# X-rayLaser/DistributedLLM

Measured on NVIDIA H100. Metric: decode tokens/sec LLaMA-7B Q4_0 seq512 bs1, higher is better.
Workload: dtype q4_0*q8_0->f32

## Files before the change

distributedllm_b200/csrc/common.cuh:

```cuda
#pragma once
#include <cuda_runtime.h>
#include <cuda_fp16.h>
#include <cstdint>
#include <cstdio>
#include <cstdarg>
#include <string>

#include "../../include/b200_slice.h"

namespace b200 {

inline std::string & last_error_ref() { static thread_local std::string e; return e; }
inline int fail(int code, const char * fmt, ...) {
    char buf[1024];
    va_list ap; va_start(ap, fmt); vsnprintf(buf, sizeof buf, fmt, ap); va_end(ap);
    last_error_ref() = buf;
    return code;
}
#define B200_CUDA(expr) do { cudaError_t e_ = (expr); if (e_ != cudaSuccess) \
    return b200::fail(B200_ECUDA, "%s failed: %s (%s:%d)", #expr, cudaGetErrorString(e_), __FILE__, __LINE__); } while (0)

__device__ __forceinline__ float fmul(float a, float b) { return __fmul_rn(a, b); }
__device__ __forceinline__ float fadd(float a, float b) { return __fadd_rn(a, b); }
__device__ __forceinline__ float fsub(float a, float b) { return __fsub_rn(a, b); }
__device__ __forceinline__ float ffma(float a, float b, float c) { return __fmaf_rn(a, b, c); }
__device__ __forceinline__ float h2f(uint16_t h) { return __half2float(__ushort_as_half(h)); }
__device__ __forceinline__ uint16_t f2h(float f) { return __half_as_ushort(__float2half_rn(f)); }

__device__ __forceinline__ uint32_t smem_u32(const void * p) { return (uint32_t) __cvta_generic_to_shared(p); }

__device__ __forceinline__ void mbar_init(uint64_t * bar, uint32_t count) {
    asm volatile("mbarrier.init.shared::cta.b64 [%0], %1;" :: "r"(smem_u32(bar)), "r"(count) : "memory");
}
__device__ __forceinline__ void mbar_fence_init() {
    asm volatile("fence.mbarrier_init.release.cluster;" ::: "memory");
}
__device__ __forceinline__ void mbar_arrive(uint64_t * bar) {
    asm volatile("{ .reg .b64 st; mbarrier.arrive.shared::cta.b64 st, [%0]; }" :: "r"(smem_u32(bar)) : "memory");
}
__device__ __forceinline__ void mbar_arrive_expect_tx(uint64_t * bar, uint32_t bytes) {
    asm volatile("{ .reg .b64 st; mbarrier.arrive.expect_tx.shared::cta.b64 st, [%0], %1; }"
                 :: "r"(smem_u32(bar)), "r"(bytes) : "memory");
}
__device__ __forceinline__ bool mbar_try_wait(uint64_t * bar, uint32_t parity) {
    uint32_t ok;
    asm volatile("{ .reg .pred p; mbarrier.try_wait.parity.shared::cta.b64 p, [%1], %2; selp.u32 %0, 1, 0, p; }"
                 : "=r"(ok) : "r"(smem_u32(bar)), "r"(parity) : "memory");
    return ok != 0;
}
__device__ __forceinline__ void mbar_wait(uint64_t * bar, uint32_t parity) {
    while (!mbar_try_wait(bar, parity)) { }
}
__device__ __forceinline__ void bulk_g2s(void * dst_smem, const void * src_gmem, uint32_t bytes, uint64_t * bar) {
    uint64_t pol;
    asm volatile("createpolicy.fractional.L2::evict_first.b64 %0, 1.0;" : "=l"(pol));
    asm volatile("cp.async.bulk.shared::cluster.global.mbarrier::complete_tx::bytes.L2::cache_hint [%0], [%1], %2, [%3], %4;"
                 :: "r"(smem_u32(dst_smem)), "l"(src_gmem), "r"(bytes), "r"(smem_u32(bar)), "l"(pol) : "memory");
}
__device__ __forceinline__ float4 ldg_keep(const float * p) {
    uint64_t pol; float4 v;
    asm volatile("createpolicy.fractional.L2::evict_last.b64 %0, 1.0;" : "=l"(pol));
    asm volatile("ld.global.L2::cache_hint.v4.f32 {%0, %1, %2, %3}, [%4], %5;"
                 : "=f"(v.x), "=f"(v.y), "=f"(v.z), "=f"(v.w) : "l"(p), "l"(pol));
    return v;
}
__device__ __forceinline__ void grid_dep_wait()   { asm volatile("griddepcontrol.wait;" ::: "memory"); }
__device__ __forceinline__ void grid_dep_launch() { asm volatile("griddepcontrol.launch_dependents;" ::: "memory"); }

__device__ __forceinline__ unsigned long long gtime() { unsigned long long t; asm volatile("mov.u64 %0, %%globaltimer;" : "=l"(t)); return t; }
#define B200_TRACE(ptr, slot) do { if (ptr) (ptr)[((size_t) blockIdx.y * gridDim.x + blockIdx.x) * 8 + (slot)] = b200::gtime(); } while (0)

__device__ __forceinline__ void named_bar_sync(int id, int nthreads) {
    asm volatile("bar.sync %0, %1;" :: "r"(id), "r"(nthreads) : "memory");
}

}
```

distributedllm_b200/csrc/fastgemm2.cuh:

```cuda
#pragma once
#include <cuda.h>

#include "kernels.cuh"

namespace b200 {

struct PrepArgs { const float * x; int ldx; const float * norm_w; uint16_t * xh; int K, N; };

template <bool NORM>
__global__ void __launch_bounds__(256) k_prep_q8_f16(const PrepArgs a) {
    __shared__ double red[8];
    grid_dep_wait();
    const int n = blockIdx.x, tid = threadIdx.x, warp = tid >> 5, lane = tid & 31;
    const float * x = a.x + (size_t) n * a.ldx;
    float scale = 1.f;
    if (NORM) {
        double s = 0.0;
        for (int i = tid; i < a.K; i += 256) s += (double) fmul(x[i], x[i]);
        for (int o = 16; o > 0; o >>= 1) s += __shfl_xor_sync(0xffffffffu, s, o);
        if (lane == 0) red[warp] = s;
        __syncthreads();
        double tot = 0.0;
        for (int i = 0; i < 8; i++) tot += red[i];
        scale = __fdiv_rn(1.0f, __fsqrt_rn(fadd((float)(tot / (double) a.K), 1e-6f)));
    }
    for (int b = warp; b < a.K / 32; b += 8) {
        float v = x[b * 32 + lane];
        if (NORM) v = fmul(fmul(v, scale), a.norm_w[b * 32 + lane]);
        float amax = fabsf(v);
        for (int o = 16; o > 0; o >>= 1) amax = fmaxf(amax, __shfl_xor_sync(0xffffffffu, amax, o));
        const float d = h2f(f2h(__fdiv_rn(amax, 127.f)));
        const float id = amax != 0.f ? __fdiv_rn(127.f, amax) : 0.f;
        const float q = (float) rint_small(fmul(v, id));
        a.xh[(size_t) n * a.K + b * 32 + lane] = f2h(fmul(q, d));
    }
}

__device__ __forceinline__ uint64_t gmma_desc_k_sw128(uint32_t smem_addr) {
    return (uint64_t)((smem_addr & 0x3FFFF) >> 4) | ((uint64_t) 1 << 16) | ((uint64_t) 64 << 32) | ((uint64_t) 1 << 62);
}
__device__ __forceinline__ void fence_proxy_async() { asm volatile("fence.proxy.async.shared::cta;" ::: "memory"); }
__device__ __forceinline__ void wgmma_fence()  { asm volatile("wgmma.fence.sync.aligned;" ::: "memory"); }
__device__ __forceinline__ void wgmma_commit() { asm volatile("wgmma.commit_group.sync.aligned;" ::: "memory"); }
template <int N> __device__ __forceinline__ void wgmma_wait() { asm volatile("wgmma.wait_group.sync.aligned %0;" :: "n"(N) : "memory"); }
__device__ __forceinline__ void acc_fence(float (&d)[64]) {
    #pragma unroll
    for (int i = 0; i < 64; i++) asm volatile("" : "+f"(d[i]) :: "memory");
}
__device__ __forceinline__ void wgmma_m64n128k16(float (&d)[64], uint64_t da, uint64_t db) {
    asm volatile("{ .reg .pred p; setp.ne.b32 p, %66, 0;\n"
                 "wgmma.mma_async.sync.aligned.m64n128k16.f32.f16.f16 {"
                 "%0, %1, %2, %3, %4, %5, %6, %7, %8, %9, %10, %11, %12, %13, %14, %15, "
                 "%16, %17, %18, %19, %20, %21, %22, %23, %24, %25, %26, %27, %28, %29, %30, %31, "
                 "%32, %33, %34, %35, %36, %37, %38, %39, %40, %41, %42, %43, %44, %45, %46, %47, "
                 "%48, %49, %50, %51, %52, %53, %54, %55, %56, %57, %58, %59, %60, %61, %62, %63}, "
                 "%64, %65, p, 1, 1, 0, 0; }"
                 : "+f"(d[0]), "+f"(d[1]), "+f"(d[2]), "+f"(d[3]), "+f"(d[4]), "+f"(d[5]), "+f"(d[6]), "+f"(d[7]),
                   "+f"(d[8]), "+f"(d[9]), "+f"(d[10]), "+f"(d[11]), "+f"(d[12]), "+f"(d[13]), "+f"(d[14]), "+f"(d[15]),
                   "+f"(d[16]), "+f"(d[17]), "+f"(d[18]), "+f"(d[19]), "+f"(d[20]), "+f"(d[21]), "+f"(d[22]), "+f"(d[23]),
                   "+f"(d[24]), "+f"(d[25]), "+f"(d[26]), "+f"(d[27]), "+f"(d[28]), "+f"(d[29]), "+f"(d[30]), "+f"(d[31]),
                   "+f"(d[32]), "+f"(d[33]), "+f"(d[34]), "+f"(d[35]), "+f"(d[36]), "+f"(d[37]), "+f"(d[38]), "+f"(d[39]),
                   "+f"(d[40]), "+f"(d[41]), "+f"(d[42]), "+f"(d[43]), "+f"(d[44]), "+f"(d[45]), "+f"(d[46]), "+f"(d[47]),
                   "+f"(d[48]), "+f"(d[49]), "+f"(d[50]), "+f"(d[51]), "+f"(d[52]), "+f"(d[53]), "+f"(d[54]), "+f"(d[55]),
                   "+f"(d[56]), "+f"(d[57]), "+f"(d[58]), "+f"(d[59]), "+f"(d[60]), "+f"(d[61]), "+f"(d[62]), "+f"(d[63])
                 : "l"(da), "l"(db), "n"(1)
                 : "memory");
}

enum { FG_STORE = 0, FG_RESID = 1, FG_GATE = 2 };

template <int EPI, class Args>
__device__ __forceinline__ void gmma_epilogue(const Args & a, const float (&d)[64], int mt, int m0, int tok0) {
    #pragma unroll
    for (int j = 0; j < 16; j++) {
        #pragma unroll
        for (int c = 0; c < 2; c++) {
            const int tok = tok0 + 8 * j + c;
            if (tok >= a.N) continue;
            if (EPI == FG_GATE) {
                const int row = (mt * 8 + (m0 >> 4)) * 8 + (m0 & 7);
                if (row < a.out_rows) a.y[(size_t) tok * a.ldy + row] = fmul(h2f(a.tsilu[f2h(d[4 * j + c])]), d[4 * j + 2 + c]);
            } else {
                #pragma unroll
                for (int i = 0; i < 2; i++) {
                    const int row = mt * 128 + m0 + 8 * i;
                    float val = d[4 * j + 2 * i + c];
                    if (row < a.out_rows) {
                        if (EPI == FG_RESID) val = fadd(val, a.resid[(size_t) tok * a.ldr + row]);
                        a.y[(size_t) tok * a.ldy + row] = val;
                    }
                }
            }
        }
    }
}

constexpr int kF2M = 128, kF2K = 128;
constexpr int kF2DqWarps = 8;
constexpr int kF2Threads = (kF2DqWarps + 1) * 32;
constexpr int kF2ABytes = kF2M * kF2K * 2;
__host__ __device__ constexpr int f2_raw_bytes(int wt) { return 16 * chunk_bytes(wt); }
__host__ __device__ constexpr int f2_stage_bytes(int wt, int nt) { return ((f2_raw_bytes(wt) + 1023) & ~1023) + kF2ABytes + nt * kF2K * 2; }
__host__ __device__ constexpr int f2_stages(int wt, int nt) { return (nt == 128 && wt == kWT_Q4_0) ? 3 : 2; }
__host__ __device__ constexpr int f2_smem(int wt, int nt) { return f2_stages(wt, nt) * f2_stage_bytes(wt, nt) + 128; }

struct FastGemm2Args {
    PackedW W;
    const float * resid; int ldr;
    float * y; int ldy;
    int N, out_rows;
    const uint16_t * tsilu;
};

__device__ __forceinline__ void tma_load_2d(void * dst, const CUtensorMap * map, int c0, int c1, uint64_t * bar) {
    asm volatile("cp.async.bulk.tensor.2d.shared::cluster.global.mbarrier::complete_tx::bytes [%0], [%1, {%2, %3}], [%4];"
                 :: "r"(smem_u32(dst)), "l"(map), "r"(c0), "r"(c1), "r"(smem_u32(bar)) : "memory");
}

template <int WT, int EPI, int NT>
__global__ void __launch_bounds__(kF2Threads, 1) k_gemm_tc2(const FastGemm2Args a, const __grid_constant__ CUtensorMap xmap) {
    constexpr int CB = (WT == kWT_Q4_0) ? kQ4Chunk : kQ8Chunk;
    constexpr int kF2N = NT, kF2BBytes = NT * kF2K * 2, kF2Stages = f2_stages(WT, NT);
    constexpr int RAW = 16 * CB, RAWP = (RAW + 1023) & ~1023, STAGE = RAWP + kF2ABytes + kF2BBytes;
    extern __shared__ __align__(1024) uint8_t smem[];
    uint64_t * bars = (uint64_t *)(smem + kF2Stages * STAGE);
    uint64_t * tma_full = bars, * stage_free = bars + 3;
    const int tid = threadIdx.x, warp = tid >> 5, lane = tid & 31;
    const int mt = blockIdx.x, nt = blockIdx.y;
    const int nbq = a.W.nbq;
    const int TRp = a.W.TR;
    const int tiles_per_m = 16 / TRp;

    if (tid == 0) {
        for (int s = 0; s < kF2Stages; s++) { mbar_init(&tma_full[s], 1); mbar_init(&stage_free[s], 2); }
        mbar_fence_init();
    }
    __syncthreads();

    if (warp == kF2DqWarps) {
        if (lane == 0) {
            grid_dep_launch();
            grid_dep_wait();
            const uint32_t per_tile = (uint32_t) TRp * CB;
            for (int kb = 0; kb < nbq; kb++) {
                const int s = kb % kF2Stages, use = kb / kF2Stages;
                if (use > 0) mbar_wait(&stage_free[s], (use - 1) & 1);
                uint8_t * stage = smem + (size_t) s * STAGE;
                mbar_arrive_expect_tx(&tma_full[s], (uint32_t)(RAW + kF2BBytes));
                for (int t = 0; t < tiles_per_m; t++) {
                    const uint8_t * src = a.W.data + (long long)(mt * tiles_per_m + t) * a.W.tile_bytes + (size_t) kb * per_tile;
                    bulk_g2s(stage + (size_t) t * per_tile, src, per_tile, &tma_full[s]);
                }
                uint8_t * B = stage + RAWP + kF2ABytes;
                tma_load_2d(B, &xmap, kb * kF2K, nt * kF2N, &tma_full[s]);
                tma_load_2d(B + kF2N * 128, &xmap, kb * kF2K + 64, nt * kF2N, &tma_full[s]);
            }
        }
    } else {
        const int wg = warp >> 2;
        float acc[NT / 128][64];
        #pragma unroll
        for (int n = 0; n < NT / 128; n++)
            #pragma unroll
            for (int i = 0; i < 64; i++) acc[n][i] = 0.f;
        const int r8 = lane >> 2, w = lane & 3;
        for (int kb = 0; kb < nbq; kb++) {
            const int s = kb % kF2Stages, use = kb / kF2Stages;
            uint8_t * stage = smem + (size_t) s * STAGE;
            uint8_t * A = stage + RAWP;
            mbar_wait(&tma_full[s], use & 1);
            #pragma unroll
            for (int gi = 0; gi < 2; gi++) {
                const int g = warp * 2 + gi;
                const uint8_t * ch = stage + (size_t) g * CB;
                const uint4 wv = *(const uint4 *)(ch + lane * 16);
                uint4 wv2 = make_uint4(0, 0, 0, 0); uint2 sc;
                if (WT == kWT_Q8_0) { wv2 = *(const uint4 *)(ch + 512 + lane * 16); sc = *(const uint2 *)(ch + 1024 + r8 * 8); }
                else sc = *(const uint2 *)(ch + 512 + r8 * 8);
                const uint32_t ww[4] = {wv.x, wv.y, wv.z, wv.w};
                const uint32_t ww2[4] = {wv2.x, wv2.y, wv2.z, wv2.w};
                const uint32_t sw[2] = {sc.x, sc.y};
                const int row = g * 8 + r8;
                #pragma unroll
                for (int bq = 0; bq < 4; bq++) {
                    const uint32_t dh = (sw[bq >> 1] >> (16 * (bq & 1))) & 0xFFFFu;
                    const __half2 d2 = __halves2half2(__ushort_as_half((unsigned short) dh), __ushort_as_half((unsigned short) dh));
                    uint32_t lo0, lo1, hi0, hi1;
                    if (WT == kWT_Q4_0) {
                        const uint32_t x = ww[bq] ^ 0x88888888u;
                        const __half2 off = __halves2half2(__ushort_as_half((unsigned short) 0x6408), __ushort_as_half((unsigned short) 0x6408));
                        uint32_t h[4];
                        #pragma unroll
                        for (int i = 0; i < 4; i++) {
                            const uint32_t m = ((x >> (4 * i)) & 0x000F000Fu) | 0x64006400u;
                            const __half2 v = __hmul2(__hsub2(*(const __half2 *) &m, off), d2);
                            h[i] = *(const uint32_t *) &v;
                        }
                        lo0 = __byte_perm(h[0], h[2], 0x5410); lo1 = __byte_perm(h[0], h[2], 0x7632);
                        hi0 = __byte_perm(h[1], h[3], 0x5410); hi1 = __byte_perm(h[1], h[3], 0x7632);
                    } else {
                        const __half2 off = __halves2half2(__ushort_as_half((unsigned short) 0x6480), __ushort_as_half((unsigned short) 0x6480));
                        const uint32_t ul = ww[bq] ^ 0x80808080u, uh = ww2[bq] ^ 0x80808080u;
                        const uint32_t m0 = __byte_perm(ul, 0x64646464u, 0x4140), m1 = __byte_perm(ul, 0x64646464u, 0x4342);
                        const uint32_t m2 = __byte_perm(uh, 0x64646464u, 0x4140), m3 = __byte_perm(uh, 0x64646464u, 0x4342);
                        const __half2 v0 = __hmul2(__hsub2(*(const __half2 *) &m0, off), d2), v1 = __hmul2(__hsub2(*(const __half2 *) &m1, off), d2);
                        const __half2 v2 = __hmul2(__hsub2(*(const __half2 *) &m2, off), d2), v3 = __hmul2(__hsub2(*(const __half2 *) &m3, off), d2);
                        lo0 = *(const uint32_t *) &v0; lo1 = *(const uint32_t *) &v1; hi0 = *(const uint32_t *) &v2; hi1 = *(const uint32_t *) &v3;
                    }
                    const int klo = bq * 32 + 4 * w, khi = klo + 16;
                    {
                        const int sub = klo >> 6, kk = klo & 63, c8 = kk >> 3, within = (kk & 7) * 2;
                        *(uint2 *)(A + sub * (kF2M * 128) + row * 128 + ((c8 ^ (row & 7)) << 4) + within) = make_uint2(lo0, lo1);
                    }
                    {
                        const int sub = khi >> 6, kk = khi & 63, c8 = kk >> 3, within = (kk & 7) * 2;
                        *(uint2 *)(A + sub * (kF2M * 128) + row * 128 + ((c8 ^ (row & 7)) << 4) + within) = make_uint2(hi0, hi1);
                    }
                }
            }
            fence_proxy_async();
            named_bar_sync(1 + wg, 128);
            const uint32_t a_addr = smem_u32(A) + wg * (64 * 128), b_addr = smem_u32(stage + RAWP + kF2ABytes);
            wgmma_fence();
            #pragma unroll
            for (int n = 0; n < NT / 128; n++) acc_fence(acc[n]);
            #pragma unroll
            for (int k16 = 0; k16 < 8; k16++) {
                const uint32_t off = (k16 & 3) * 32;
                #pragma unroll
                for (int n = 0; n < NT / 128; n++)
                    wgmma_m64n128k16(acc[n], gmma_desc_k_sw128(a_addr + (k16 >> 2) * (kF2M * 128) + off),
                                     gmma_desc_k_sw128(b_addr + (k16 >> 2) * (kF2N * 128) + n * (128 * 128) + off));
            }
            wgmma_commit();
            wgmma_wait<1>();
            #pragma unroll
            for (int n = 0; n < NT / 128; n++) acc_fence(acc[n]);
            if (kb > 0 && (tid & 127) == 0) mbar_arrive(&stage_free[(kb - 1) % kF2Stages]);
        }
        wgmma_wait<0>();
        #pragma unroll
        for (int n = 0; n < NT / 128; n++) acc_fence(acc[n]);
        #pragma unroll
        for (int n = 0; n < NT / 128; n++)
            gmma_epilogue<EPI>(a, acc[n], mt, wg * 64 + (warp & 3) * 16 + r8, nt * kF2N + n * 128 + 2 * w);
    }
}

}
```

distributedllm_b200/csrc/kernels.cuh:

```cuda
#pragma once
#include "common.cuh"

namespace b200 {

constexpr int kWT_F16 = 1, kWT_Q4_0 = 2, kWT_Q4_1 = 3, kWT_Q5_0 = 6, kWT_Q5_1 = 7, kWT_Q8_0 = 8;
constexpr int kQ4Chunk = 576, kQ41Chunk = 640, kQ50Chunk = 704, kQ51Chunk = 768, kQ8Chunk = 1088;
constexpr int kWPC = 4;
constexpr int kConsumers = kWPC * 32;
constexpr int kQS = 4;
constexpr float kMagic = 12582912.0f;
constexpr int kMagicI = 0x4B400000;

struct WtTraits {
    int block_bytes;
    int chunk_bytes;
    bool is_signed;
    bool min_plane;
    bool high_plane;
    bool q8_1;
    float act_scale;
};
__host__ __device__ constexpr WtTraits wt_traits(int wt) {
    return wt == kWT_Q4_0 ? WtTraits{18, kQ4Chunk, true, false, false, false, 0.0625f}
         : wt == kWT_Q4_1 ? WtTraits{20, kQ41Chunk, false, true, false, true, 0.0625f}
// ... 153 lines not shown
}

enum { PRO_PLAIN = 0, PRO_NORM = 1, PRO_PREQ = 2 };
enum { EPI_STORE = 0, EPI_RESID = 1, EPI_GATE = 2, EPI_GATEQ = 3, EPI_RESID_NQ = 4, EPI_RESID_SEND = 5 };

struct GemvArgs {
    PackedW W;
    const float * x;      int ldx;
    const float * norm_w;
    const int * aq_in; const float * da_in;
    int in_soff, out_soff;
    const float * resid;  int ldr;
    float * y;            int ldy;
    int * aq_out; float * da_out; int out_nbq; float out_dscale;
    const float * nq_norm_w; int * nq_counter; double * nq_partial;
    int N;
    int out_rows;
    const uint16_t * tsilu;
    int NS;
    unsigned long long * trace;
    int pre_stages;
    int dbg_nomath;
    MailboxHdr * mb_mine;
    uint2 * mb_peer_inbox; size_t mb_slot_elems;
};

__host__ __device__ inline size_t act_bytes_per_col(int nbq, int wt) { return (size_t) nbq * (128 + 16 + (wt_q8_1(wt) ? 16 : 0)); }


__device__ __forceinline__ double widen_nonneg(float f) {
    const uint32_t u = __float_as_uint(f);
    if (u - 0x00800000u < 0x7F000000u) return __hiloint2double((int)((u >> 3) + 0x38000000u), (int)(u << 29));
    return (double) f;
}
__device__ __forceinline__ int rint_small(float x) { return __float_as_int(fadd(x, kMagic)) - kMagicI; }

__device__ __forceinline__ int dp4a_us(uint32_t a, int b, int c) {
    int d; asm("dp4a.u32.s32 %0, %1, %2, %3;" : "=r"(d) : "r"(a), "r"(b), "r"(c)); return d;
}

__device__ __forceinline__ void warp_quant_block(float v, int lane, int * aq_col, float * da_col, int b, float dscale, int soff = 0) {
    float amax = fabsf(v);
    #pragma unroll
    for (int o = 16; o > 0; o >>= 1) amax = fmaxf(amax, __shfl_xor_sync(0xffffffffu, amax, o));
    const float dq = __fdiv_rn(amax, 127.f);
    const float d = soff ? dq : h2f(f2h(dq));
    const float id = amax != 0.f ? __fdiv_rn(127.f, amax) : 0.f;
    const int qv = rint_small(fmul(v, id));
    uint32_t pk = ((uint32_t)(qv & 0xFF)) << (8 * (lane & 3));
    pk |= __shfl_xor_sync(0xffffffffu, pk, 1);
    pk |= __shfl_xor_sync(0xffffffffu, pk, 2);
    if ((lane & 3) == 0) {
        const int w = lane >> 2;
        aq_col[(b >> 2) * 32 + (w & 3) * 8 + (b & 3) * 2 + (w >> 2)] = (int) pk;
    }
    if (lane == 0) da_col[b] = fmul(d, dscale);
    if (soff) {
        int qs = qv;
        #pragma unroll
        for (int o = 16; o > 0; o >>= 1) qs += __shfl_xor_sync(0xffffffffu, qs, o);
        if (lane == 0) da_col[soff + b] = fmul(d, (float) qs);
    }
}

template <int WT>
__device__ __forceinline__ void thread_quant_block(const float (&v)[32], int * an, float * dn, int b, int rot = 0, float * sn = nullptr) {
    constexpr bool Q81 = wt_q8_1(WT);
    float m[8];
    #pragma unroll
    for (int j = 0; j < 8; j++) m[j] = fmaxf(fmaxf(fabsf(v[j]), fabsf(v[j + 8])), fmaxf(fabsf(v[j + 16]), fabsf(v[j + 24])));
    const float amax = fmaxf(fmaxf(fmaxf(m[0], m[1]), fmaxf(m[2], m[3])), fmaxf(fmaxf(m[4], m[5]), fmaxf(m[6], m[7])));
    const float dq = __fdiv_rn(amax, 127.f);
    const float d = Q81 ? dq : h2f(f2h(dq));
    const float id = amax != 0.f ? __fdiv_rn(127.f, amax) : 0.f;
    dn[b] = wt_nibbles(WT) ? fmul(d, wt_act_scale(WT)) : d;
    int * dst = an + (b >> 2) * 32 + (b & 3) * 2;
    int qsum = 0;
    #pragma unroll
    for (int w = 0; w < 8; w++) {
        uint32_t pk = 0;
        #pragma unroll
        for (int j = 0; j < 4; j++) {
            const int qv = rint_small(fmul(v[w*4 + j], id));
            if (Q81) qsum += qv;
            pk |= ((uint32_t)(qv & 0xFF)) << (8 * j);
        }
        const int ww = (w + rot) & 7;
        dst[(ww & 3) * 8 + (ww >> 2)] = (int) pk;
    }
    if (Q81) sn[b] = fmul(d, (float) qsum);
}

template <int WT, int G, int NC, int PRO, int EPI, bool RING>
__global__ void __launch_bounds__(kConsumers + 32) k_gemv(const GemvArgs a) {
    constexpr int CB = chunk_bytes(WT);
    constexpr bool Q41 = wt_q8_1(WT);
    constexpr bool Q5 = wt_traits(WT).high_plane;
    constexpr int SOFF = wt_scale_off(WT), MOFF = wt_min_off(WT);
    constexpr int TR = kWPC * G;
    extern __shared__ __align__(128) uint8_t smem[];
    const int nbq = a.W.nbq, K = a.W.K, nb = a.W.nb;
    const int NS = a.NS;
    constexpr int stage_bytes = kQS * TR * CB;
    uint8_t * ring = smem;
    int * a_s = (int *)(smem + (RING ? (size_t) NS * stage_bytes : 0));
    float * da_s = (float *)((uint8_t *) a_s + (size_t) NC * nbq * 128);
    float * sa_s = da_s + (size_t) NC * nbq * 4;
    uint64_t * full = (uint64_t *)((uint8_t *) da_s + (size_t) NC * nbq * (Q41 ? 32 : 16));
    uint64_t * empty = full + 16;
    uint64_t * actbar = empty + 16;
    double * red = (double *)(actbar + 2);
    float * gq = (float *)(red + kWPC);
    float * xs = gq + NC * 32;

    const int tid = threadIdx.x, warp = tid >> 5, lane = tid & 31;
    const int col0 = blockIdx.y * NC;
    const int n_stage = nbq / kQS;

    if (tid == 0) {
        B200_TRACE(a.trace, 0);
        if (RING) for (int s = 0; s < NS; s++) { mbar_init(&full[s], 1); mbar_init(&empty[s], kWPC); }
        mbar_init(actbar, 1);
        mbar_init(actbar + 1, kWPC);
        mbar_fence_init();
    }
    __syncthreads();

    if (RING && warp == kWPC) {
        if (lane == 0) {
            int slot = 0, use = 0, issued = 0;
            for (int tile = blockIdx.x; tile < a.W.n_tiles; tile += gridDim.x) {
                const uint8_t * src = a.W.data + (long long) tile * a.W.tile_bytes;
                for (int s = 0; s < n_stage; s++) {
                    if (issued == a.pre_stages) mbar_wait(actbar + 1, 0);
                    issued++;
                    if (use > 0) mbar_wait(&empty[slot], (use - 1) & 1);
                    mbar_arrive_expect_tx(&full[slot], (uint32_t) stage_bytes);
                    bulk_g2s(ring + (size_t) slot * stage_bytes, src + (size_t) s * stage_bytes, (uint32_t) stage_bytes, &full[slot]);
                    if (++slot == NS) { slot = 0; use++; }
                }
            }
            if (issued <= a.pre_stages) mbar_wait(actbar + 1, 0);
            grid_dep_launch();
            B200_TRACE(a.trace, 4);
        }
        return;
    }

    float wn[32];
    if (PRO == PRO_NORM && nb <= kConsumers) {
        #pragma unroll
        for (int j = 0; j < 8; j++) {
            const float4 u = tid < nb ? ldg_keep(a.norm_w + tid * 32 + (((NC == 1 ? tid : 0) + j) & 7) * 4) : make_float4(0.f, 0.f, 0.f, 0.f);
            wn[j*4] = u.x; wn[j*4+1] = u.y; wn[j*4+2] = u.z; wn[j*4+3] = u.w;
        }
    }
    grid_dep_wait();
    if (!RING && tid == 0) grid_dep_launch();
    if (tid == 0) B200_TRACE(a.trace, 1);

    const int ncols = min(NC, a.N - col0);
    bool gate_done = false;
    if (PRO == PRO_PREQ) {
        gate_done = true;
        if (tid == 0) {
            const uint32_t b1 = (uint32_t) ncols * nbq * 128, b2 = (uint32_t) ncols * nbq * 16;
            mbar_arrive_expect_tx(actbar, b1 + b2 + (Q41 ? b2 : 0u));
            bulk_g2s(a_s, a.aq_in + (size_t) col0 * nbq * 32, b1, actbar);
            bulk_g2s(da_s, a.da_in + (size_t) col0 * nbq * 4, b2, actbar);
            if (Q41) bulk_g2s(sa_s, a.da_in + a.in_soff + (size_t) col0 * nbq * 4, b2, actbar);
        }
        if (RING && lane == 0) mbar_arrive(actbar + 1);
        for (int n = ncols; n < NC; n++) {
            for (int i = tid; i < nbq * 32; i += kConsumers) a_s[(size_t) n * nbq * 32 + i] = 0;
            for (int i = tid; i < nbq * 4; i += kConsumers) { da_s[(size_t) n * nbq * 4 + i] = 0.f; if (Q41) sa_s[(size_t) n * nbq * 4 + i] = 0.f; }
        }
        mbar_wait(actbar, 0);
    } else {
        for (int n = 0; n < NC; n++) {
            int * an = a_s + (size_t) n * nbq * 32;
            float * dn = da_s + (size_t) n * nbq * 4;
            float * sn = sa_s + (size_t) n * nbq * 4;
            if (n >= ncols) {
                for (int i = tid; i < nbq * 32; i += kConsumers) an[i] = 0;
                for (int i = tid; i < nbq * 4; i += kConsumers) { dn[i] = 0.f; if (Q41) sn[i] = 0.f; }
                continue;
            }
            const float * x = a.x + (size_t)(col0 + n) * a.ldx;
            for (int b = nb + tid; b < nbq * 4; b += kConsumers) {
                int * dst = an + (b >> 2) * 32 + (b & 3) * 2;
                for (int w = 0; w < 4; w++) { dst[w * 8] = 0; dst[w * 8 + 1] = 0; }
                dn[b] = 0.f;
                if (Q41) sn[b] = 0.f;
            }
            if (PRO == PRO_NORM && nb <= kConsumers) {
                float v[32];
                const bool own = tid < nb;
                const int rot = NC == 1 ? (tid & 7) : 0;
                if (NC == 1) {
                    if (tid == 0) { mbar_arrive_expect_tx(actbar, (uint32_t) K * 4); bulk_g2s(xs, x, (uint32_t) K * 4, actbar); }
                    if (RING && lane == 0) { gate_done = true; mbar_arrive(actbar + 1); }
                    mbar_wait(actbar, 0);
                    #pragma unroll
                    for (int j = 0; j < 8; j++) {
                        const float4 t = own ? *(const float4 *)(xs + tid * 32 + ((j + rot) & 7) * 4) : make_float4(0.f, 0.f, 0.f, 0.f);
                        v[j*4] = t.x; v[j*4+1] = t.y; v[j*4+2] = t.z; v[j*4+3] = t.w;
                    }
                } else {
                    #pragma unroll
                    for (int j = 0; j < 8; j++) {
                        const float4 t = own ? *(const float4 *)(x + tid * 32 + j * 4) : make_float4(0.f, 0.f, 0.f, 0.f);
                        v[j*4] = t.x; v[j*4+1] = t.y; v[j*4+2] = t.z; v[j*4+3] = t.w;
                    }
                    if (RING && n == ncols - 1 && lane == 0) { gate_done = true; mbar_arrive(actbar + 1); }
                }
                double s4[4] = {0.0, 0.0, 0.0, 0.0};
                #pragma unroll
                for (int j = 0; j < 32; j++) s4[j & 3] += widen_nonneg(fmul(v[j], v[j]));
                double s = (s4[0] + s4[1]) + (s4[2] + s4[3]);
                if (tid == 0) B200_TRACE(a.trace, 5);
                for (int o = 16; o > 0; o >>= 1) s += __shfl_xor_sync(0xffffffffu, s, o);
                if (lane == 0) red[warp] = s;
                named_bar_sync(1, kConsumers);
                const double tot = (red[0] + red[1]) + (red[2] + red[3]);
                named_bar_sync(1, kConsumers);
                const float scale = __fdiv_rn(1.0f, __fsqrt_rn(fadd((float)(tot / (double) K), 1e-6f)));
                if (tid == 0) B200_TRACE(a.trace, 6);
                if (own) {
                    #pragma unroll
                    for (int j = 0; j < 32; j++) v[j] = fmul(fmul(v[j], scale), wn[j]);
                    thread_quant_block<WT>(v, an, dn, tid, rot, sn);
                }
            } else {
                float scale = 1.0f;
                if (PRO == PRO_NORM) {
                    double s = 0.0;
                    for (int i = tid * 4; i < K; i += kConsumers * 4) {
                        const float4 v = *(const float4 *)(x + i);
                        s += (double) fmul(v.x, v.x); s += (double) fmul(v.y, v.y);
                        s += (double) fmul(v.z, v.z); s += (double) fmul(v.w, v.w);
                    }
                    for (int o = 16; o > 0; o >>= 1) s += __shfl_xor_sync(0xffffffffu, s, o);
                    if (lane == 0) red[warp] = s;
                    named_bar_sync(1, kConsumers);
                    const double tot = (red[0] + red[1]) + (red[2] + red[3]);
                    named_bar_sync(1, kConsumers);
                    scale = __fdiv_rn(1.0f, __fsqrt_rn(fadd((float)(tot / (double) K), 1e-6f)));
                }
                for (int b = tid; b < nb; b += kConsumers) {
                    float v[32];
                    #pragma unroll
                    for (int j = 0; j < 8; j++) {
                        float4 t = *(const float4 *)(x + b * 32 + j * 4);
                        if (PRO == PRO_NORM) {
                            const float4 wv = *(const float4 *)(a.norm_w + b * 32 + j * 4);
                            t.x = fmul(fmul(t.x, scale), wv.x); t.y = fmul(fmul(t.y, scale), wv.y);
                            t.z = fmul(fmul(t.z, scale), wv.z); t.w = fmul(fmul(t.w, scale), wv.w);
                        }
                        v[j*4] = t.x; v[j*4+1] = t.y; v[j*4+2] = t.z; v[j*4+3] = t.w;
                    }
                    thread_quant_block<WT>(v, an, dn, b, 0, sn);
                }
            }
        }
    }
    if (RING && lane == 0 && !gate_done) mbar_arrive(actbar + 1);
    named_bar_sync(1, kConsumers);
    if (tid == 0) B200_TRACE(a.trace, 2);

    const int r = lane >> 2, w = lane & 3;
    int slot = 0, phase = 0;
#ifdef B200_TRACE_WAITS
    long long dbg_wait = 0, dbg_t0 = a.trace ? clock64() : 0;
#endif
    uint2 * send_slot = nullptr; int send_seq = 0;
    if (EPI == EPI_RESID_SEND) {
        send_seq = a.mb_mine->seq_out + 1;
        if (lane == 0) mb_wait_slot_free(a.mb_mine, send_seq);
        __syncwarp();
        send_slot = a.mb_peer_inbox + (size_t)(send_seq & (kMbSlots - 1)) * a.mb_slot_elems;
    }
    for (int tile = blockIdx.x; tile < a.W.n_tiles; tile += gridDim.x) {
        float acc[G][NC][2];
        float summ[G][NC];
        #pragma unroll
        for (int g = 0; g < G; g++)
            #pragma unroll
            for (int n = 0; n < NC; n++) { acc[g][n][0] = 0.f; acc[g][n][1] = 0.f; summ[g][n] = 0.f; }
        const uint8_t * gsrc = a.W.data + (long long) tile * a.W.tile_bytes;

        for (int s = 0; s < n_stage; s++) {
            const uint8_t * base;
            if (RING) {
#ifdef B200_TRACE_WAITS
                if (a.trace) { const long long c0 = clock64(); mbar_wait(&full[slot], phase); dbg_wait += clock64() - c0; }
                else
#endif
                mbar_wait(&full[slot], phase);
                base = ring + (size_t) slot * stage_bytes;
            } else {
                base = gsrc + (size_t) s * stage_bytes;
            }
            base += (size_t)(warp * G) * CB;
            if (!a.dbg_nomath)
            #pragma unroll
            for (int qi = 0; qi < kQS; qi++) {
                const int Q = s * kQS + qi;
                uint4 wv[G], wv2[G]; uint2 sc[G], mc[G]; uint32_t hw[G];
                #pragma unroll
                for (int g = 0; g < G; g++) {
                    const uint8_t * ch = base + (size_t)(qi * TR + g) * CB;
                    wv[g] = *(const uint4 *)(ch + lane * 16);
                    if (WT == kWT_Q8_0) wv2[g] = *(const uint4 *)(ch + 512 + lane * 16);
                    sc[g] = *(const uint2 *)(ch + SOFF + r * 8);
                    mc[g] = Q41 ? *(const uint2 *)(ch + MOFF + r * 8) : make_uint2(0u, 0u);
                    hw[g] = Q5 ? *(const uint32_t *)(ch + 512 + lane * 4) : 0u;
                }
                #pragma unroll
                for (int n = 0; n < NC; n++) {
                    const int4 * ap = (const int4 *)(a_s + (size_t) n * nbq * 32 + Q * 32 + w * 8);
                    const int4 a01 = ap[0], a23 = ap[1];
                    const float4 dav = *(const float4 *)(da_s + (size_t) n * nbq * 4 + Q * 4);
                    const int alo[4] = {a01.x, a01.z, a23.x, a23.z};
                    const int ahi[4] = {a01.y, a01.w, a23.y, a23.w};
                    const float da[4] = {dav.x, dav.y, dav.z, dav.w};
                    float sa[4] = {0.f, 0.f, 0.f, 0.f};
                    if (Q41) { const float4 sav = *(const float4 *)(sa_s + (size_t) n * nbq * 4 + Q * 4); sa[0] = sav.x; sa[1] = sav.y; sa[2] = sav.z; sa[3] = sav.w; }
                    #pragma unroll
                    for (int g = 0; g < G; g++) {
                        const uint32_t ww[4] = {wv[g].x, wv[g].y, wv[g].z, wv[g].w};
                        const uint32_t ww2[4] = {wv2[g].x, wv2[g].y, wv2[g].z, wv2[g].w};
                        const uint32_t sw[2] = {sc[g].x, sc[g].y};
                        const uint32_t mw[2] = {mc[g].x, mc[g].y};
                        #pragma unroll
                        for (int bq = 0; bq < 4; bq++) {
                            const uint16_t dh = (uint16_t)(sw[bq >> 1] >> (16 * (bq & 1)));
                            const float D = fmul(h2f(dh), da[bq]);
                            float f0, f1;
                            if (Q41) {
                                const uint16_t mh = (uint16_t)(mw[bq >> 1] >> (16 * (bq & 1)));
                                summ[g][n] = fadd(summ[g][n], fmul(h2f(mh), sa[bq]));
                                uint32_t lo, hi;
                                if (Q5) {
                                    lo = ((ww[bq] << 3) & 0x78787878u) | spread4_hi((hw[g] >> (8 * bq)) & 15u);
                                    hi = ((ww[bq] >> 1) & 0x78787878u) | spread4_hi((hw[g] >> (8 * bq + 4)) & 15u);
                                } else { lo = (ww[bq] << 4) & 0xF0F0F0F0u; hi = ww[bq] & 0xF0F0F0F0u; }
                                f0 = fadd(__int_as_float(dp4a_us(lo, alo[bq], kMagicI)), -kMagic);
                                f1 = fadd(__int_as_float(dp4a_us(hi, ahi[bq], kMagicI)), -kMagic);
                            } else {
                                int lo, hi;
                                if (WT == kWT_Q4_0) { lo = (int)((ww[bq] << 4) & 0xF0F0F0F0u); hi = (int)(ww[bq] & 0xF0F0F0F0u); }
                                else if (Q5) {
                                    lo = (int)(((ww[bq] << 3) & 0x78787878u) | (spread4_hi((hw[g] >> (8 * bq)) & 15u) ^ 0x80808080u));
                                    hi = (int)(((ww[bq] >> 1) & 0x78787878u) | (spread4_hi((hw[g] >> (8 * bq + 4)) & 15u) ^ 0x80808080u));
                                }
                                else                { lo = (int) ww[bq]; hi = (int) ww2[bq]; }
                                f0 = fadd(__int_as_float(__dp4a(lo, alo[bq], kMagicI)), -kMagic);
                                f1 = fadd(__int_as_float(__dp4a(hi, ahi[bq], kMagicI)), -kMagic);
                            }
                            acc[g][n][0] = ffma(D, f0, acc[g][n][0]);
                            acc[g][n][1] = ffma(D, f1, acc[g][n][1]);
                        }
                    }
                }
            }
            if (RING) {
                __syncwarp();
                if (lane == 0) mbar_arrive(&empty[slot]);
                if (++slot == NS) { slot = 0; phase ^= 1; }
            }
        }

        float res[G][NC];
        #pragma unroll
        for (int g = 0; g < G; g++)
            #pragma unroll
            for (int n = 0; n < NC; n++) {
                float t = fadd(acc[g][n][0], acc[g][n][1]);
                t = fadd(t, __shfl_xor_sync(0xffffffffu, t, 2));
                t = fadd(t, __shfl_xor_sync(0xffffffffu, t, 1));
                res[g][n] = Q41 ? fadd(t, summ[g][n]) : t;
            }
        if (EPI == EPI_GATE || EPI == EPI_GATEQ) {
            const int row = (tile * kWPC + warp) * 8 + r;
            if (w == 0) {
                #pragma unroll
                for (int n = 0; n < NC; n++) {
                    const float gv = fmul(h2f(a.tsilu[f2h(res[0][n])]), res[G - 1][n]);
                    if (EPI == EPI_GATEQ) gq[n * 32 + warp * 8 + r] = row < a.out_rows ? gv : 0.f;
                    else if (row < a.out_rows && n < ncols) a.y[(size_t)(col0 + n) * a.ldy + row] = gv;
                }
            }
            if (EPI == EPI_GATEQ) {
                named_bar_sync(1, kConsumers);
                for (int n = warp; n < ncols; n += kWPC)
                    warp_quant_block(gq[n * 32 + lane], lane, a.aq_out + (size_t)(col0 + n) * a.out_nbq * 32,
                                     a.da_out + (size_t)(col0 + n) * a.out_nbq * 4, tile, a.out_dscale, a.out_soff);
                named_bar_sync(1, kConsumers);
            }
        } else if (w == 0) {
            #pragma unroll
            for (int g = 0; g < G; g++) {
                const int row = ((tile * kWPC + warp) * G + g) * 8 + r;
                if (row < a.out_rows) {
                    #pragma unroll
                    for (int n = 0; n < NC; n++) {
                        if (n < ncols) {
                            float v = res[g][n];
                            if (EPI == EPI_RESID || EPI == EPI_RESID_NQ || EPI == EPI_RESID_SEND) v = fadd(v, a.resid[(size_t)(col0 + n) * a.ldr + row]);
                            a.y[(size_t)(col0 + n) * a.ldy + row] = v;
                            if (EPI == EPI_RESID_SEND) st_ll(send_slot + row, v, send_seq);
                            if (EPI == EPI_RESID_NQ) gq[n * 32 + warp * 8 + r] = v;
                        }
                    }
                }
            }
        }
    }
    if (EPI == EPI_RESID_NQ) {
        named_bar_sync(1, kConsumers);
        if (warp == 0) {
            const int tile = blockIdx.x, nt = (int) gridDim.x;
            for (int n = 0; n < ncols; n++) {
                const float val = gq[n * 32 + lane];
                double s = widen_nonneg(fmul(val, val));
                for (int o = 16; o > 0; o >>= 1) s += __shfl_xor_sync(0xffffffffu, s, o);
                double * part = a.nq_partial + ((size_t) blockIdx.y * NC + n) * nt;
                if (lane == 0) part[tile] = s;
            }
            int * cnt = a.nq_counter + 2 * blockIdx.y;
            if (lane == 0) {
                __threadfence();
                atomicAdd(cnt, 1);
                while (*(volatile int *) cnt < nt) { }
                __threadfence();
            }
            __syncwarp();
            const int row = tile * 32 + lane;
            for (int n = 0; n < ncols; n++) {
                const double * part = a.nq_partial + ((size_t) blockIdx.y * NC + n) * nt;
                double s = 0.0;
                for (int i = lane; i < nt; i += 32) s += __ldcg(part + i);
                for (int o = 16; o > 0; o >>= 1) s += __shfl_xor_sync(0xffffffffu, s, o);
                const float scale = __fdiv_rn(1.0f, __fsqrt_rn(fadd((float)(s / (double) a.out_rows), 1e-6f)));
                const float val = gq[n * 32 + lane];
                const float wv = row < a.out_rows ? a.nq_norm_w[row] : 0.f;
                warp_quant_block(fmul(fmul(val, scale), wv), lane, a.aq_out + (size_t)(col0 + n) * a.out_nbq * 32,
                                 a.da_out + (size_t)(col0 + n) * a.out_nbq * 4, tile, a.out_dscale, a.out_soff);
            }
            if (lane == 0) {
                if (atomicAdd(cnt + 1, 1) == nt - 1) { cnt[0] = 0; cnt[1] = 0; }
            }
        }
    }
    if (tid == 0) B200_TRACE(a.trace, 3);
#ifdef B200_TRACE_WAITS
    if (tid == 0 && a.trace)
        a.trace[((size_t) blockIdx.y * gridDim.x + blockIdx.x) * 8 + 7] = ((unsigned long long) dbg_wait << 32) | (unsigned long long)((clock64() - dbg_t0) & 0xFFFFFFFFll);
#endif
}

struct NormQuantArgs {
    const float * x; int ldx; const float * norm_w; int K;
    int * aq; float * da; int nbq;
    int soff;
};

template <int WT>
__global__ void __launch_bounds__(256) k_norm_quant(const NormQuantArgs a) {
    __shared__ double red[8];
    const int n = blockIdx.x, tid = threadIdx.x, warp = tid >> 5, lane = tid & 31, nb = a.K / 32;
    if (tid == 0) grid_dep_launch();
    grid_dep_wait();
    const float * x = a.x + (size_t) n * a.ldx;
    double s = 0.0;
    for (int b = tid; b < nb; b += 256) {
        #pragma unroll
        for (int j = 0; j < 8; j++) {
            const float4 t = *(const float4 *)(x + b * 32 + j * 4);
            s += widen_nonneg(fmul(t.x, t.x)); s += widen_nonneg(fmul(t.y, t.y));
            s += widen_nonneg(fmul(t.z, t.z)); s += widen_nonneg(fmul(t.w, t.w));
        }
    }
    for (int o = 16; o > 0; o >>= 1) s += __shfl_xor_sync(0xffffffffu, s, o);
    if (lane == 0) red[warp] = s;
    __syncthreads();
    double tot = 0.0;
    #pragma unroll
    for (int i = 0; i < 8; i++) tot += red[i];
    const float scale = __fdiv_rn(1.0f, __fsqrt_rn(fadd((float)(tot / (double) a.K), 1e-6f)));
    int * an = a.aq + (size_t) n * a.nbq * 32;
    float * dn = a.da + (size_t) n * a.nbq * 4;
    for (int b = tid; b < nb; b += 256) {
        float v[32];
        #pragma unroll
        for (int j = 0; j < 8; j++) {
            const float4 t = *(const float4 *)(x + b * 32 + j * 4);
            const float4 wv = *(const float4 *)(a.norm_w + b * 32 + j * 4);
            v[j*4]   = fmul(fmul(t.x, scale), wv.x); v[j*4+1] = fmul(fmul(t.y, scale), wv.y);
            v[j*4+2] = fmul(fmul(t.z, scale), wv.z); v[j*4+3] = fmul(fmul(t.w, scale), wv.w);
        }
        thread_quant_block<WT>(v, an, dn, b, 0, dn + a.soff);
    }
}

struct GemvF16Args {
    const uint16_t * W;
    const uint16_t * tail;
    int rows, K;
    const float * x; int ldx; const float * norm_w;
    const float * resid; int ldr;
    float * y; int ldy; int N;
    const uint16_t * tsilu;
    const uint16_t * W2; const uint16_t * tail2;
};

template <int PRO, int EPI>
__global__ void __launch_bounds__(256) k_gemv_f16(const GemvF16Args a) {
    extern __shared__ __align__(16) uint8_t smem[];
    uint16_t * xh = (uint16_t *) smem;
    __shared__ double red[8];
    const int tid = threadIdx.x, warp = tid >> 5, lane = tid & 31, K = a.K;
    const int col = blockIdx.y;
    grid_dep_wait();
    const float * x = a.x + (size_t) col * a.ldx;
    float scale = 1.0f;
    if (PRO == PRO_NORM) {
        double s = 0.0;
        for (int i = tid; i < K; i += 256) s += (double) fmul(x[i], x[i]);
        for (int o = 16; o > 0; o >>= 1) s += __shfl_xor_sync(0xffffffffu, s, o);
        if (lane == 0) red[warp] = s;
        __syncthreads();
        double tot = 0.0;
        for (int i = 0; i < 8; i++) tot += red[i];
        scale = __fdiv_rn(1.0f, __fsqrt_rn(fadd((float)(tot / (double) K), 1e-6f)));
    }
    for (int i = tid; i < K; i += 256) {
        float v = x[i];
        if (PRO == PRO_NORM) v = fmul(fmul(v, scale), a.norm_w[i]);
        xh[i] = f2h(v);
    }
    __syncthreads();
    const int nchunk = K / 32, nc8 = (nchunk + 7) / 8, ntail = K & 31;
    for (int row = blockIdx.x * 8 + warp; row < a.rows; row += gridDim.x * 8) {
        float res[2] = {0.f, 0.f};
        #pragma unroll
        for (int m = 0; m < (EPI == EPI_GATE ? 2 : 1); m++) {
            const uint16_t * Wm = m ? a.W2 : a.W;
            const uint16_t * tl = m ? a.tail2 : a.tail;
            float acc = 0.f;
            const uint4 * wp = (const uint4 *)(Wm + ((size_t) row * nc8 * 32 + lane) * 8);
            constexpr int U = 4;
            for (int c8 = 0; c8 < nc8; c8 += U) {
                uint4 v[U];
                #pragma unroll
                for (int q = 0; q < U; q++) v[q] = c8 + q < nc8 ? __ldcs(wp + (size_t)(c8 + q) * 32) : make_uint4(0, 0, 0, 0);
                #pragma unroll
                for (int q = 0; q < U; q++) {
                    const uint32_t u[4] = {v[q].x, v[q].y, v[q].z, v[q].w};
                    #pragma unroll
                    for (int j = 0; j < 8; j++) {
                        const int c = (c8 + q) * 8 + j;
                        if (c < nchunk) {
                            const uint16_t wh = (uint16_t)(u[j >> 1] >> (16 * (j & 1)));
                            acc = ffma(h2f(wh), h2f(xh[c * 32 + lane]), acc);
                        }
                    }
                }
            }
            acc = fadd(acc, __shfl_xor_sync(0xffffffffu, acc, 16));
            acc = fadd(acc, __shfl_xor_sync(0xffffffffu, acc, 8));
            acc = fadd(acc, __shfl_xor_sync(0xffffffffu, acc, 4));
            acc = fadd(acc, __shfl_xor_sync(0xffffffffu, acc, 1));
            acc = fadd(acc, __shfl_xor_sync(0xffffffffu, acc, 2));
            double sumf = (double) acc;
            for (int i = 0; i < ntail; i++)
                sumf += (double) fmul(h2f(tl[(size_t) row * ntail + i]), h2f(xh[nchunk * 32 + i]));
            res[m] = (float) sumf;
        }
        if (lane == 0) {
            float v = res[0];
            if (EPI == EPI_RESID) v = fadd(v, a.resid[(size_t) col * a.ldr + row]);
            if (EPI == EPI_GATE)  v = fmul(h2f(a.tsilu[f2h(res[0])]), res[1]);
            a.y[(size_t) col * a.ldy + row] = v;
        }
    }
}

template <int PRO, int EPI, int NC>
__global__ void __launch_bounds__(256) k_gemv_f16_mc(const GemvF16Args a) {
    static_assert(NC == 4 || NC == 8, "columns per CTA");
    extern __shared__ __align__(16) uint8_t smem[];
    float * xf = (float *) smem;
    __shared__ double red[8];
    const int tid = threadIdx.x, warp = tid >> 5, lane = tid & 31, K = a.K;
    const int col0 = blockIdx.y * NC, ncols = min(NC, a.N - col0);
    grid_dep_wait();
    for (int n = 0; n < NC; n++) {
        if (n >= ncols) { for (int i = tid; i < K; i += 256) xf[(size_t) i * NC + n] = 0.f; continue; }
        const float * x = a.x + (size_t)(col0 + n) * a.ldx;
        float scale = 1.0f;
        if (PRO == PRO_NORM) {
            double s = 0.0;
            for (int i = tid; i < K; i += 256) s += (double) fmul(x[i], x[i]);
            for (int o = 16; o > 0; o >>= 1) s += __shfl_xor_sync(0xffffffffu, s, o);
            __syncthreads();
            if (lane == 0) red[warp] = s;
            __syncthreads();
            double tot = 0.0;
            for (int i = 0; i < 8; i++) tot += red[i];
            scale = __fdiv_rn(1.0f, __fsqrt_rn(fadd((float)(tot / (double) K), 1e-6f)));
        }
        for (int i = tid; i < K; i += 256) {
            float v = x[i];
            if (PRO == PRO_NORM) v = fmul(fmul(v, scale), a.norm_w[i]);
            xf[(size_t) i * NC + n] = h2f(f2h(v));
        }
    }
    __syncthreads();
    const int nchunk = K / 32, nc8 = (nchunk + 7) / 8, ntail = K & 31;
    for (int row0 = (blockIdx.x * 8 + warp) * 2; row0 < a.rows; row0 += gridDim.x * 16) {
        const bool two = row0 + 1 < a.rows;
        float res[2][2][NC];
        #pragma unroll
        for (int m = 0; m < (EPI == EPI_GATE ? 2 : 1); m++) {
            const uint16_t * Wm = m ? a.W2 : a.W;
            const uint16_t * tl = m ? a.tail2 : a.tail;
            float acc[2][NC];
            #pragma unroll
            for (int n = 0; n < NC; n++) { acc[0][n] = 0.f; acc[1][n] = 0.f; }
            const uint4 * wp0 = (const uint4 *)(Wm + ((size_t) row0 * nc8 * 32 + lane) * 8);
            const uint4 * wp1 = (const uint4 *)(Wm + ((size_t)(two ? row0 + 1 : row0) * nc8 * 32 + lane) * 8);
            constexpr int U = 2;
            uint4 v0[U], v1[U];
            #pragma unroll
            for (int q = 0; q < U; q++) {
                v0[q] = q < nc8 ? __ldg(wp0 + (size_t) q * 32) : make_uint4(0, 0, 0, 0);
                v1[q] = q < nc8 ? __ldg(wp1 + (size_t) q * 32) : make_uint4(0, 0, 0, 0);
            }
            for (int c8 = 0; c8 < nc8; c8 += U) {
                uint4 n0[U], n1[U];
                #pragma unroll
                for (int q = 0; q < U; q++) {
                    n0[q] = c8 + U + q < nc8 ? __ldg(wp0 + (size_t)(c8 + U + q) * 32) : make_uint4(0, 0, 0, 0);
                    n1[q] = c8 + U + q < nc8 ? __ldg(wp1 + (size_t)(c8 + U + q) * 32) : make_uint4(0, 0, 0, 0);
                }
                #pragma unroll
                for (int q = 0; q < U; q++) {
                    const uint32_t u0[4] = {v0[q].x, v0[q].y, v0[q].z, v0[q].w};
                    const uint32_t u1[4] = {v1[q].x, v1[q].y, v1[q].z, v1[q].w};
                    #pragma unroll
                    for (int j = 0; j < 8; j++) {
                        const int c = (c8 + q) * 8 + j;
                        if (c < nchunk) {
                            const float w0 = h2f((uint16_t)(u0[j >> 1] >> (16 * (j & 1))));
                            const float w1 = h2f((uint16_t)(u1[j >> 1] >> (16 * (j & 1))));
                            const float4 * xp = (const float4 *)(xf + (size_t)(c * 32 + lane) * NC);
                            #pragma unroll
                            for (int n4 = 0; n4 < NC / 4; n4++) {
                                const float4 xv = xp[n4];
                                acc[0][n4*4]   = ffma(w0, xv.x, acc[0][n4*4]);   acc[0][n4*4+1] = ffma(w0, xv.y, acc[0][n4*4+1]);
                                acc[0][n4*4+2] = ffma(w0, xv.z, acc[0][n4*4+2]); acc[0][n4*4+3] = ffma(w0, xv.w, acc[0][n4*4+3]);
                                acc[1][n4*4]   = ffma(w1, xv.x, acc[1][n4*4]);   acc[1][n4*4+1] = ffma(w1, xv.y, acc[1][n4*4+1]);
                                acc[1][n4*4+2] = ffma(w1, xv.z, acc[1][n4*4+2]); acc[1][n4*4+3] = ffma(w1, xv.w, acc[1][n4*4+3]);
                            }
                        }
                    }
                }
                #pragma unroll
                for (int q = 0; q < U; q++) { v0[q] = n0[q]; v1[q] = n1[q]; }
            }
            #pragma unroll
            for (int rr = 0; rr < 2; rr++)
// ... 808 lines not shown
```

Measured before the change: 554.3.

## Release ring slot early after batching shared-memory weight loads in GEMV

For the single-column (decode) ring-buffered path, each warp now loads several quant groups of weights from the shared-memory stage into registers at once. It then releases the stage's empty barrier, with a proxy fence, before doing the math on the last group. This lets the producer's bulk copy into that slot start sooner and overlap with the remaining compute. The cost is higher register pressure from holding LQ groups of weights live, which could lower occupancy.

```diff
diff --git a/distributedllm_b200/csrc/common.cuh b/distributedllm_b200/csrc/common.cuh
--- a/distributedllm_b200/csrc/common.cuh
+++ b/distributedllm_b200/csrc/common.cuh
@@ -42,6 +42,7 @@
     asm volatile("{ .reg .b64 st; mbarrier.arrive.expect_tx.shared::cta.b64 st, [%0], %1; }"
                  :: "r"(smem_u32(bar)), "r"(bytes) : "memory");
 }
+__device__ __forceinline__ void fence_proxy_async() { asm volatile("fence.proxy.async.shared::cta;" ::: "memory"); }
 __device__ __forceinline__ bool mbar_try_wait(uint64_t * bar, uint32_t parity) {
     uint32_t ok;
     asm volatile("{ .reg .pred p; mbarrier.try_wait.parity.shared::cta.b64 p, [%1], %2; selp.u32 %0, 1, 0, p; }"
diff --git a/distributedllm_b200/csrc/fastgemm2.cuh b/distributedllm_b200/csrc/fastgemm2.cuh
--- a/distributedllm_b200/csrc/fastgemm2.cuh
+++ b/distributedllm_b200/csrc/fastgemm2.cuh
@@ -39,7 +39,6 @@
 __device__ __forceinline__ uint64_t gmma_desc_k_sw128(uint32_t smem_addr) {
     return (uint64_t)((smem_addr & 0x3FFFF) >> 4) | ((uint64_t) 1 << 16) | ((uint64_t) 64 << 32) | ((uint64_t) 1 << 62);
 }
-__device__ __forceinline__ void fence_proxy_async() { asm volatile("fence.proxy.async.shared::cta;" ::: "memory"); }
 __device__ __forceinline__ void wgmma_fence()  { asm volatile("wgmma.fence.sync.aligned;" ::: "memory"); }
 __device__ __forceinline__ void wgmma_commit() { asm volatile("wgmma.commit_group.sync.aligned;" ::: "memory"); }
 template <int N> __device__ __forceinline__ void wgmma_wait() { asm volatile("wgmma.wait_group.sync.aligned %0;" :: "n"(N) : "memory"); }
diff --git a/distributedllm_b200/csrc/kernels.cuh b/distributedllm_b200/csrc/kernels.cuh
--- a/distributedllm_b200/csrc/kernels.cuh
+++ b/distributedllm_b200/csrc/kernels.cuh
@@ -479,73 +479,83 @@
                 base = gsrc + (size_t) s * stage_bytes;
             }
             base += (size_t)(warp * G) * CB;
-            if (!a.dbg_nomath)
-            #pragma unroll
-            for (int qi = 0; qi < kQS; qi++) {
-                const int Q = s * kQS + qi;
-                uint4 wv[G], wv2[G]; uint2 sc[G], mc[G]; uint32_t hw[G];
-                #pragma unroll
-                for (int g = 0; g < G; g++) {
-                    const uint8_t * ch = base + (size_t)(qi * TR + g) * CB;
-                    wv[g] = *(const uint4 *)(ch + lane * 16);
-                    if (WT == kWT_Q8_0) wv2[g] = *(const uint4 *)(ch + 512 + lane * 16);
-                    sc[g] = *(const uint2 *)(ch + SOFF + r * 8);
-                    mc[g] = Q41 ? *(const uint2 *)(ch + MOFF + r * 8) : make_uint2(0u, 0u);
-                    hw[g] = Q5 ? *(const uint32_t *)(ch + 512 + lane * 4) : 0u;
-                }
-                #pragma unroll
-                for (int n = 0; n < NC; n++) {
-                    const int4 * ap = (const int4 *)(a_s + (size_t) n * nbq * 32 + Q * 32 + w * 8);
-                    const int4 a01 = ap[0], a23 = ap[1];
-                    const float4 dav = *(const float4 *)(da_s + (size_t) n * nbq * 4 + Q * 4);
-                    const int alo[4] = {a01.x, a01.z, a23.x, a23.z};
-                    const int ahi[4] = {a01.y, a01.w, a23.y, a23.w};
-                    const float da[4] = {dav.x, dav.y, dav.z, dav.w};
-                    float sa[4] = {0.f, 0.f, 0.f, 0.f};
-                    if (Q41) { const float4 sav = *(const float4 *)(sa_s + (size_t) n * nbq * 4 + Q * 4); sa[0] = sav.x; sa[1] = sav.y; sa[2] = sav.z; sa[3] = sav.w; }
-                    #pragma unroll
-                    for (int g = 0; g < G; g++) {
-                        const uint32_t ww[4] = {wv[g].x, wv[g].y, wv[g].z, wv[g].w};
-                        const uint32_t ww2[4] = {wv2[g].x, wv2[g].y, wv2[g].z, wv2[g].w};
-                        const uint32_t sw[2] = {sc[g].x, sc[g].y};
-                        const uint32_t mw[2] = {mc[g].x, mc[g].y};
-                        #pragma unroll
-                        for (int bq = 0; bq < 4; bq++) {
-                            const uint16_t dh = (uint16_t)(sw[bq >> 1] >> (16 * (bq & 1)));
-                            const float D = fmul(h2f(dh), da[bq]);
-                            float f0, f1;
-                            if (Q41) {
-                                const uint16_t mh = (uint16_t)(mw[bq >> 1] >> (16 * (bq & 1)));
-                                summ[g][n] = fadd(summ[g][n], fmul(h2f(mh), sa[bq]));
-                                uint32_t lo, hi;
-                                if (Q5) {
-                                    lo = ((ww[bq] << 3) & 0x78787878u) | spread4_hi((hw[g] >> (8 * bq)) & 15u);
-                                    hi = ((ww[bq] >> 1) & 0x78787878u) | spread4_hi((hw[g] >> (8 * bq + 4)) & 15u);
-                                } else { lo = (ww[bq] << 4) & 0xF0F0F0F0u; hi = ww[bq] & 0xF0F0F0F0u; }
-                                f0 = fadd(__int_as_float(dp4a_us(lo, alo[bq], kMagicI)), -kMagic);
-                                f1 = fadd(__int_as_float(dp4a_us(hi, ahi[bq], kMagicI)), -kMagic);
-                            } else {
-                                int lo, hi;
-                                if (WT == kWT_Q4_0) { lo = (int)((ww[bq] << 4) & 0xF0F0F0F0u); hi = (int)(ww[bq] & 0xF0F0F0F0u); }
-                                else if (Q5) {
-                                    lo = (int)(((ww[bq] << 3) & 0x78787878u) | (spread4_hi((hw[g] >> (8 * bq)) & 15u) ^ 0x80808080u));
-                                    hi = (int)(((ww[bq] >> 1) & 0x78787878u) | (spread4_hi((hw[g] >> (8 * bq + 4)) & 15u) ^ 0x80808080u));
-                                }
-                                else                { lo = (int) ww[bq]; hi = (int) ww2[bq]; }
-                                f0 = fadd(__int_as_float(__dp4a(lo, alo[bq], kMagicI)), -kMagic);
-                                f1 = fadd(__int_as_float(__dp4a(hi, ahi[bq], kMagicI)), -kMagic);
-                            }
-                            acc[g][n][0] = ffma(D, f0, acc[g][n][0]);
-                            acc[g][n][1] = ffma(D, f1, acc[g][n][1]);
-                        }
-                    }
-                }
-            }
-            if (RING) {
+            constexpr bool early = RING && NC == 1;
+            constexpr int LQ = early ? kQS / G : 1;
+            auto release = [&] {
+                if (early) fence_proxy_async();
                 __syncwarp();
                 if (lane == 0) mbar_arrive(&empty[slot]);
                 if (++slot == NS) { slot = 0; phase ^= 1; }
-            }
+            };
+            if (!a.dbg_nomath)
+            #pragma unroll
+            for (int q0 = 0; q0 < kQS; q0 += LQ) {
+                uint4 wv[LQ][G], wv2[LQ][G]; uint2 sc[LQ][G], mc[LQ][G]; uint32_t hw[LQ][G];
+                #pragma unroll
+                for (int l = 0; l < LQ; l++)
+                    #pragma unroll
+                    for (int g = 0; g < G; g++) {
+                        const uint8_t * ch = base + (size_t)((q0 + l) * TR + g) * CB;
+                        wv[l][g] = *(const uint4 *)(ch + lane * 16);
+                        if (WT == kWT_Q8_0) wv2[l][g] = *(const uint4 *)(ch + 512 + lane * 16);
+                        sc[l][g] = *(const uint2 *)(ch + SOFF + r * 8);
+                        mc[l][g] = Q41 ? *(const uint2 *)(ch + MOFF + r * 8) : make_uint2(0u, 0u);
+                        hw[l][g] = Q5 ? *(const uint32_t *)(ch + 512 + lane * 4) : 0u;
+                    }
+                #pragma unroll
+                for (int l = 0; l < LQ; l++) {
+                    const int Q = s * kQS + q0 + l;
+                    if (early && q0 + LQ == kQS && l == LQ - 1) release();
+                    #pragma unroll
+                    for (int n = 0; n < NC; n++) {
+                        const int4 * ap = (const int4 *)(a_s + (size_t) n * nbq * 32 + Q * 32 + w * 8);
+                        const int4 a01 = ap[0], a23 = ap[1];
+                        const float4 dav = *(const float4 *)(da_s + (size_t) n * nbq * 4 + Q * 4);
+                        const int alo[4] = {a01.x, a01.z, a23.x, a23.z};
+                        const int ahi[4] = {a01.y, a01.w, a23.y, a23.w};
+                        const float da[4] = {dav.x, dav.y, dav.z, dav.w};
+                        float sa[4] = {0.f, 0.f, 0.f, 0.f};
+                        if (Q41) { const float4 sav = *(const float4 *)(sa_s + (size_t) n * nbq * 4 + Q * 4); sa[0] = sav.x; sa[1] = sav.y; sa[2] = sav.z; sa[3] = sav.w; }
+                        #pragma unroll
+                        for (int g = 0; g < G; g++) {
+                            const uint32_t ww[4] = {wv[l][g].x, wv[l][g].y, wv[l][g].z, wv[l][g].w};
+                            const uint32_t ww2[4] = {wv2[l][g].x, wv2[l][g].y, wv2[l][g].z, wv2[l][g].w};
+                            const uint32_t sw[2] = {sc[l][g].x, sc[l][g].y};
+                            const uint32_t mw[2] = {mc[l][g].x, mc[l][g].y};
+                            #pragma unroll
+                            for (int bq = 0; bq < 4; bq++) {
+                                const uint16_t dh = (uint16_t)(sw[bq >> 1] >> (16 * (bq & 1)));
+                                const float D = fmul(h2f(dh), da[bq]);
+                                float f0, f1;
+                                if (Q41) {
+                                    const uint16_t mh = (uint16_t)(mw[bq >> 1] >> (16 * (bq & 1)));
+                                    summ[g][n] = fadd(summ[g][n], fmul(h2f(mh), sa[bq]));
+                                    uint32_t lo, hi;
+                                    if (Q5) {
+                                        lo = ((ww[bq] << 3) & 0x78787878u) | spread4_hi((hw[l][g] >> (8 * bq)) & 15u);
+                                        hi = ((ww[bq] >> 1) & 0x78787878u) | spread4_hi((hw[l][g] >> (8 * bq + 4)) & 15u);
+                                    } else { lo = (ww[bq] << 4) & 0xF0F0F0F0u; hi = ww[bq] & 0xF0F0F0F0u; }
+                                    f0 = fadd(__int_as_float(dp4a_us(lo, alo[bq], kMagicI)), -kMagic);
+                                    f1 = fadd(__int_as_float(dp4a_us(hi, ahi[bq], kMagicI)), -kMagic);
+                                } else {
+                                    int lo, hi;
+                                    if (WT == kWT_Q4_0) { lo = (int)((ww[bq] << 4) & 0xF0F0F0F0u); hi = (int)(ww[bq] & 0xF0F0F0F0u); }
+                                    else if (Q5) {
+                                        lo = (int)(((ww[bq] << 3) & 0x78787878u) | (spread4_hi((hw[l][g] >> (8 * bq)) & 15u) ^ 0x80808080u));
+                                        hi = (int)(((ww[bq] >> 1) & 0x78787878u) | (spread4_hi((hw[l][g] >> (8 * bq + 4)) & 15u) ^ 0x80808080u));
+                                    }
+                                    else                { lo = (int) ww[bq]; hi = (int) ww2[bq]; }
+                                    f0 = fadd(__int_as_float(__dp4a(lo, alo[bq], kMagicI)), -kMagic);
+                                    f1 = fadd(__int_as_float(__dp4a(hi, ahi[bq], kMagicI)), -kMagic);
+                                }
+                                acc[g][n][0] = ffma(D, f0, acc[g][n][0]);
+                                acc[g][n][1] = ffma(D, f1, acc[g][n][1]);
+                            }
+                        }
+                    }
+                }
+            }
+            if (RING && (!early || a.dbg_nomath)) release();
         }
 
         float res[G][NC];
```

Result: no change. 556.6, median of 6 (+0.4%).
